# mandt-lab/PSLD

Hardware: NVIDIA B200
Metric: PSLD CIFAR-10 samples/sec (SSCS sampler) (higher is better)
Workload: dtype bf16x3

## Files before the change

### psld_b200/csrc/capi.cu

```cuda

#include <stdarg.h>
#include <string.h>

#include "common.cuh"

namespace psld {

static thread_local char g_err[512] = "";

void set_error(const char* fmt, ...) {
  va_list ap;
  va_start(ap, fmt);
  vsnprintf(g_err, sizeof(g_err), fmt, ap);
  va_end(ap);
}

static int op_launch_count(const psld_op& op) {
  switch (op.kind) {
    case PSLD_OP_LAYOUT: return 1;
    case PSLD_OP_TEMB: return 4;
    case PSLD_OP_GN:
      return (op.in[4] && (op.i[PSLD_GN_C2] == 0 || op.in[5])) ? 1 : 2;
    case PSLD_OP_FIR: return 1;
    case PSLD_OP_CONV: return 1;
    case PSLD_OP_ATTN: return 1;
    case PSLD_OP_AXPBY: return 1;
    default: return 0;
  }
}

static int dispatch(const psld_op& op, cudaStream_t s) {
  switch (op.kind) {
    case PSLD_OP_LAYOUT: return run_layout(op, s);
    case PSLD_OP_TEMB: return run_temb(op, s);
    case PSLD_OP_GN: return run_gn(op, s);
    case PSLD_OP_FIR: return run_fir(op, s);
    case PSLD_OP_CONV:
      if (op.engine == PSLD_ENGINE_TC_GN) return run_conv_gn_tc(op, s);
      return op.engine == PSLD_ENGINE_TC ? run_conv_tc(op, s) : run_conv_simt(op, s);
    case PSLD_OP_ATTN:
      return op.engine == PSLD_ENGINE_TC ? run_attn_tc(op, s) : run_attn_simt(op, s);
    case PSLD_OP_AXPBY: return run_axpby(op, s);
    case PSLD_OP_ZERO: {
      const size_t bytes = (size_t)op.i[0] | ((size_t)op.i[1] << 31);
      if (bytes == 0) return PSLD_OK;
      PSLD_CHECK_ARG(op.out[0] != nullptr, "zero: null pointer");
      PSLD_CHECK_CUDA(cudaMemsetAsync(op.out[0], 0, bytes, s));
      return PSLD_OK;
    }
    default:
      set_error("unknown op kind %d", op.kind);
      return PSLD_EINVAL;
  }
}

}

using namespace psld;

extern "C" int psld_version(void) { return PSLD_B200_VERSION; }

extern "C" const char* psld_last_error(void) { return g_err; }

extern "C" int psld_device_info(int* sm_count, int* cc_major, int* cc_minor) {
  int dev = 0;
  PSLD_CHECK_CUDA(cudaGetDevice(&dev));
  cudaDeviceProp prop;
  PSLD_CHECK_CUDA(cudaGetDeviceProperties(&prop, dev));
  if (sm_count) *sm_count = prop.multiProcessorCount;
  if (cc_major) *cc_major = prop.major;
  if (cc_minor) *cc_minor = prop.minor;
  return PSLD_OK;
}

extern "C" int psld_axpby(float* out, float a, const float* x, float b, const float* y, int64_t n,
                          psld_stream_t stream) {
  return launch_axpby(out, a, x, b, y, n, (cudaStream_t)stream);
}

extern "C" int psld_op_prepare(psld_op* op) {
  PSLD_CHECK_ARG(op != nullptr, "psld_op_prepare: null op");
  if (op->kind == PSLD_OP_CONV && op->engine == PSLD_ENGINE_TC) return prepare_conv_tc(*op);
  if (op->kind == PSLD_OP_CONV && op->engine == PSLD_ENGINE_TC_GN) return prepare_conv_gn_tc(*op);
  if (op->kind == PSLD_OP_ATTN && op->engine == PSLD_ENGINE_TC) return prepare_attn_tc(*op);
  return PSLD_OK;
}

extern "C" int psld_op_release(psld_op* op) {
  PSLD_CHECK_ARG(op != nullptr, "psld_op_release: null op");
  if (op->kind == PSLD_OP_CONV && op->engine == PSLD_ENGINE_TC) return release_conv_tc(*op);
  if (op->kind == PSLD_OP_CONV && op->engine == PSLD_ENGINE_TC_GN) return release_conv_gn_tc(*op);
  if (op->kind == PSLD_OP_ATTN && op->engine == PSLD_ENGINE_TC) return release_attn_tc(*op);
  return PSLD_OK;
}

extern "C" int psld_op_run(const psld_op* op, psld_stream_t stream) {
  PSLD_CHECK_ARG(op != nullptr, "psld_op_run: null op");
  return dispatch(*op, (cudaStream_t)stream);
}

extern "C" int psld_program_run(const psld_op* ops, int n_ops, psld_stream_t stream) {
  PSLD_CHECK_ARG(ops != nullptr && n_ops >= 0, "psld_program_run: bad program");
  for (int i = 0; i < n_ops; ++i) {
    const int rc = dispatch(ops[i], (cudaStream_t)stream);
    if (rc != PSLD_OK) {
      char inner[400];
      strncpy(inner, g_err, sizeof(inner) - 1);
      inner[sizeof(inner) - 1] = 0;
      set_error("op %d (kind %d): %s", i, ops[i].kind, inner);
      return rc;
    }
  }
  return PSLD_OK;
}

extern "C" int psld_program_launches(const psld_op* ops, int n_ops) {
  if (!ops || n_ops < 0) return 0;
  int n = 0;
  for (int i = 0; i < n_ops; ++i) n += op_launch_count(ops[i]);
  return n;
}

static int run_net(const psld_op* ops, int n_ops, int temb_op, const float* time_ptr,
                   cudaStream_t s, int* step_counter = nullptr) {
  for (int i = 0; i < n_ops; ++i) {
    int rc;
    if (i == temb_op || ops[i].kind == PSLD_OP_TEMB) {
      psld_op t = ops[i];
      t.in[0] = time_ptr;
      t.out[2] = step_counter;
      rc = dispatch(t, s);
    } else {
      rc = dispatch(ops[i], s);
    }
    if (rc != PSLD_OK) return rc;
  }
  return PSLD_OK;
}

extern "C" int psld_sampler_run(const psld_op* ops, int n_ops, const psld_sampler_desc* d,
                                psld_stream_t stream) {
  PSLD_CHECK_ARG(ops && d && n_ops > 0, "psld_sampler_run: null argument");
  PSLD_CHECK_ARG(d->state && d->net_in && d->eps && d->time_table, "psld_sampler_run: null buffer");
  PSLD_CHECK_ARG(d->n_steps >= 0 && d->B > 0 && d->chw > 0 && d->chw % 4 == 0,
                 "psld_sampler_run: bad sizes");
  PSLD_CHECK_ARG(d->temb_op >= 0 && d->temb_op < n_ops && ops[d->temb_op].kind == PSLD_OP_TEMB,
                 "psld_sampler_run: temb_op does not index a TEMB op");
  PSLD_CHECK_ARG(d->sampler == 0 ? d->sscs != nullptr : d->em != nullptr,
                 "psld_sampler_run: missing coefficient table");
  PSLD_CHECK_ARG(!d->denoise || d->den, "psld_sampler_run: denoise needs coefficients");
  PSLD_CHECK_ARG(!(d->record && d->fuse_halves), "psld_sampler_run: record requires fuse_halves=0");
  cudaStream_t s = (cudaStream_t)stream;
  const int64_t per_draw = d->B * 2 * d->chw;
  const size_t state_bytes = (size_t)per_draw * dtype_size(d->state_dtype);
  auto z = [&](int64_t k) -> const float* { return d->noise ? d->noise + k * per_draw : nullptr; };
  const int n = d->n_steps;
  int rc = PSLD_OK;

  const bool graph = d->step_counter != nullptr && d->noise == nullptr && d->record == nullptr &&
                     n > 1 && (d->sampler == 0 ? d->sscs_dev != nullptr : d->em_dev != nullptr);
  if (graph) {
    PSLD_CHECK_ARG(s != nullptr, "psld_sampler_run: graph replay needs a non-default stream");
    const int fuse = d->sampler == 0 ? d->fuse_halves : 0;
    if (d->sampler == 0 && fuse && n > 0) {
      rc = psld_sscs_update(d->state, d->state, d->state_dtype, d->net_in, nullptr, nullptr, nullptr,
                            nullptr, &d->sscs[0], PSLD_STAGE_HALF_A, d->seed, 0, d->B, d->chw, s);
      if (rc) return rc;
    }
    const int n_graph = (d->sampler == 0 && fuse == 1) ? n - 1 : n;
    cudaGraph_t g = nullptr;
    cudaGraphExec_t ge = nullptr;
    PSLD_CHECK_CUDA(cudaStreamBeginCapture(s, cudaStreamCaptureModeThreadLocal));
    rc = PSLD_OK;
    if (d->sampler == 0) {
      if (!fuse)
        rc = launch_sscs_table(d->state, d->state_dtype, d->net_in, nullptr, d->sscs_dev,
                               d->step_counter, PSLD_STAGE_HALF_A, d->seed, d->B, d->chw, s);
      if (!rc) rc = run_net(ops, n_ops, d->temb_op, d->time_table, s, d->step_counter);
      int stages = PSLD_STAGE_SCORE | PSLD_STAGE_HALF_B;
      if (fuse == 1) stages |= PSLD_STAGE_HALF_C;
// ... 77 lines not shown
```

### psld_b200/csrc/common.cuh

```cuda
#pragma once

#include <cuda_bf16.h>
#include <cuda_runtime.h>
#include <stdint.h>
#include <stdio.h>

#include "../../include/psld_b200.h"

namespace psld {

void set_error(const char* fmt, ...);

#define PSLD_CHECK_ARG(cond, ...)            \
  do {                                       \
    if (!(cond)) {                           \
      ::psld::set_error(__VA_ARGS__);        \
      return PSLD_EINVAL;                    \
    }                                        \
  } while (0)

#define PSLD_CHECK_CUDA(expr)                                                          \
  do {                                                                                 \
    cudaError_t _e = (expr);                                                           \
    if (_e != cudaSuccess) {                                                           \
// ... 97 lines not shown
    split_bf2(v.x, v.y, h.x, l.x);
    split_bf2(v.z, v.w, h.y, l.y);
    *reinterpret_cast<uint2*>(p) = h;
    *reinterpret_cast<uint2*>(p + lo) = l;
  }
};

template <typename T>
__device__ __forceinline__ float ld_elt(const T* p, int lo);
template <>
__device__ __forceinline__ float ld_elt<float>(const float* p, int) { return *p; }
template <>
__device__ __forceinline__ float ld_elt<__nv_bfloat16>(const __nv_bfloat16* p, int) {
  return __bfloat162float(*p);
}
template <>
__device__ __forceinline__ float ld_elt<bf16s>(const bf16s* p, int lo) {
  return __bfloat162float(p[0].v) + __bfloat162float(p[lo].v);
}
template <typename T>
__device__ __forceinline__ void st_elt(T* p, float v, int lo);
template <>
__device__ __forceinline__ void st_elt<float>(float* p, float v, int) { *p = v; }
template <>
__device__ __forceinline__ void st_elt<__nv_bfloat16>(__nv_bfloat16* p, float v, int) {
  *p = __float2bfloat16_rn(v);
}
template <>
__device__ __forceinline__ void st_elt<bf16s>(bf16s* p, float v, int lo) {
  const __nv_bfloat16 h = __float2bfloat16_rn(v);
  p[0].v = h;
  p[lo].v = __float2bfloat16_rn(v - __bfloat162float(h));
}

template <typename T>
__device__ __forceinline__ float to_f32(T v);
template <>
__device__ __forceinline__ float to_f32<float>(float v) { return v; }
template <>
__device__ __forceinline__ float to_f32<__nv_bfloat16>(__nv_bfloat16 v) {
  return __bfloat162float(v);
}
template <typename T>
__device__ __forceinline__ T from_f32(float v);
template <>
__device__ __forceinline__ float from_f32<float>(float v) { return v; }
template <>
__device__ __forceinline__ __nv_bfloat16 from_f32<__nv_bfloat16>(float v) {
  return __float2bfloat16_rn(v);
}

__device__ __forceinline__ float silu_f(float x) { return x / (1.0f + expf(-x)); }

static inline size_t dtype_size(int dt) { return dt == PSLD_BF16 ? 2 : (dt == PSLD_F64 ? 8 : 4); }

int run_layout(const psld_op& op, cudaStream_t s);
int run_axpby(const psld_op& op, cudaStream_t s);
int launch_axpby(float* out, float a, const float* x, float b, const float* y, int64_t n,
                 cudaStream_t s);
int run_temb(const psld_op& op, cudaStream_t s);
int run_gn(const psld_op& op, cudaStream_t s);
int run_fir(const psld_op& op, cudaStream_t s);
int run_conv_simt(const psld_op& op, cudaStream_t s);
int run_attn_simt(const psld_op& op, cudaStream_t s);
int prepare_conv_tc(psld_op& op);
int release_conv_tc(psld_op& op);
int run_conv_tc(const psld_op& op, cudaStream_t s);
int prepare_conv_gn_tc(psld_op& op);
int release_conv_gn_tc(psld_op& op);
int run_conv_gn_tc(const psld_op& op, cudaStream_t s);
int prepare_attn_tc(psld_op& op);
int release_attn_tc(psld_op& op);
int run_attn_tc(const psld_op& op, cudaStream_t s);

int launch_step_inc(int* step_ptr, cudaStream_t s);
int launch_sscs_table(void* u, int state_dtype, float* net_in, const float* eps,
                      const psld_sscs_coeffs* table, const int* step_ptr, int stages, uint64_t seed,
                      int64_t B, int64_t chw, cudaStream_t s);
int launch_em_table(void* u, int state_dtype, float* net_in, const float* eps,
                    const psld_score_step* table, const int* step_ptr, uint64_t seed, int64_t B,
                    int64_t chw, cudaStream_t s);

}
```

### psld_b200/csrc/conv_gn_tc.cu

```cuda

#include <cuda.h>

#include <new>

#include "common.cuh"
#include "tc_common.cuh"
#include "conv_tc_common.cuh"

namespace psld {

constexpr int GN_TRANSFORM_WARPS = 8;
constexpr int GN_THREADS = (12 + GN_TRANSFORM_WARPS) * 32;
constexpr int GN_B_STAGES = 4;
constexpr int GN_B_BYTES = 128 * 128;
constexpr int GN_MAX_ROWS = 192;
constexpr int GN_VAR_BYTES = GN_MAX_ROWS * 128;
constexpr int GN_ABUF_BYTES = 3 * GN_VAR_BYTES;
constexpr int GN_STAGING_BYTES = 8 * 2048;
constexpr int GN_ADDV_BYTES = 8 * 256;
constexpr int GN_SMEM_BYTES = 2 * GN_ABUF_BYTES + GN_B_STAGES * GN_B_BYTES + GN_STAGING_BYTES + 256 + GN_ADDV_BYTES + 768;

struct ConvGnParams {
  ConvTcParams c;
  const float* affine;
  int cin;
  int silu;
  int rows_in;
  int w_shift;
  int n_images;
};

struct ConvGnState {
  CUtensorMap a1, a2, b, b2, e1, e2;
  ConvGnParams p;
  int grid;
  bool x3;
};

__device__ __forceinline__ int gn_tap(int t9) {
  const int kx = t9 < 3 ? 1 : (t9 < 6 ? 0 : 2);
  const int ky = t9 < 3 ? t9 : (t9 < 6 ? t9 - 3 : t9 - 6);
  return ky * 3 + kx;
}

__device__ __forceinline__ float silu_fast(float x) {
  const float h = 0.5f * x;
  float t;
  asm("tanh.approx.f32 %0, %1;" : "=f"(t) : "f"(h));
  return fmaf(h, t, h);
}

__global__ void __launch_bounds__(GN_THREADS, 1)
conv_gn_tc_kernel(const __grid_constant__ CUtensorMap tmA1, const __grid_constant__ CUtensorMap tmA2,
                  const __grid_constant__ CUtensorMap tmB, const __grid_constant__ CUtensorMap tmB2,
                  const __grid_constant__ CUtensorMap tmE1,
                  const __grid_constant__ CUtensorMap tmE2, const ConvGnParams gp) {
  const ConvTcParams& p = gp.c;
  extern __shared__ uint8_t smem_raw[];
  pdl_launch_dependents();
  const uint32_t base = (smem_u32(smem_raw) + 1023u) & ~1023u;
  auto abuf = [&](int b) { return base + (uint32_t)b * GN_ABUF_BYTES; };
  const uint32_t bring = base + 2 * GN_ABUF_BYTES;
  const uint32_t stg_base = bring + GN_B_STAGES * GN_B_BYTES;
  const uint32_t bar_base = stg_base + GN_STAGING_BYTES;
  const uint32_t addv_base = bar_base + 256u;
  if (addv_base + GN_ADDV_BYTES > smem_u32(smem_raw) + GN_SMEM_BYTES) __trap();
  auto raw_full = [&](int b) { return bar_base + 8u * b; };
  auto a_ready = [&](int b) { return bar_base + 8u * (2 + b); };
  auto a_empty = [&](int b) { return bar_base + 8u * (4 + b); };
  auto b_full = [&](int s) { return bar_base + 8u * (6 + s); };
  auto b_empty = [&](int s) { return bar_base + 8u * (6 + GN_B_STAGES + s); };
  auto tfull_bar = [&](int s) { return bar_base + 8u * (6 + 2 * GN_B_STAGES + s); };
  auto tempty_bar = [&](int s) { return bar_base + 8u * (8 + 2 * GN_B_STAGES + s); };
  auto c_empty = [&](int b) { return bar_base + 8u * (10 + 2 * GN_B_STAGES + b); };
  const uint32_t tmem_slot = bar_base + 8u * (12 + 2 * GN_B_STAGES);
  volatile uint32_t* tmem_slot_ptr =
      reinterpret_cast<volatile uint32_t*>(smem_raw + (tmem_slot - smem_u32(smem_raw)));
// ... 227 lines not shown
          }
          if (x == Wm) *sptr(R + off) = make_uint4(0u, 0u, 0u, 0u);
        }
        asm volatile("fence.proxy.async.shared::cta;" ::: "memory");
        asm volatile("bar.sync 1, %0;" ::"n"(GN_TRANSFORM_WARPS * 32) : "memory");
        if (tt == 0) mbar_arrive_remote(leader_ready0 + 8u * (uint32_t)buf);
        if (++buf == 2) { buf = 0; ph ^= 1; }
      }
    }
  } else if (warp >= 4) {
    const int quarter = warp & 3;
    const int half = (warp - 4) >> 2;
    const uint32_t leader_tempty0 = mapa_rank(tempty_bar(0), 0);
    int acc = 0;
    uint32_t acc_phase = 0;
    pdl_wait();
    for (int v = unit0; v < p.num_virtual; v += unit_step) {
        int unit, nsub, bn;
        tc_decode_unit(p, v, unit, nsub, bn);
      const int n_tile = nsub < 0 ? unit % p.n_tiles_n : (unit % p.n_tiles_n) * p.n_split + nsub;
      const int m_tile = 2 * (unit / p.n_tiles_n) + (int)rank;
      tc_epilogue_tile<true, 32, false>(
          p, tmem_base, acc, m_tile, n_tile, bn, quarter, half, lane,
          stg_base + (uint32_t)(warp - 4) * 2048u, addv_base + (uint32_t)(warp - 4) * 256u,
          [&]() {
            mbar_wait(tfull_bar(acc), acc_phase);
            tc_fence_after();
          },
          [&]() {
            tc_fence_before();
            __syncwarp();
            if (lane == 0) mbar_arrive_remote_relaxed(leader_tempty0 + 8u * (uint32_t)acc);
          });
      if (++acc == 2) { acc = 0; acc_phase ^= 1; }
    }
  }

  tc_fence_before();
  cluster_sync_all();
  if (warp == 1) {
    tc_fence_after();
    asm volatile("tcgen05.dealloc.cta_group::2.sync.aligned.b32 %0, %1;"
                 ::"r"(tmem_base), "n"(TC_TMEM_COLS) : "memory");
  }
}

constexpr int GX_THREADS = 384;
constexpr int GX_TRANSFORM_WARPS = 4;
constexpr int GX_B_STAGES = 2;
constexpr int GX_B_STAGE = 2 * GN_B_BYTES;
constexpr int GX_ABUF_BYTES = 6 * GN_VAR_BYTES;
constexpr int GX_STAGING_BYTES = 4 * 4096;
constexpr int GX_ADDV_BYTES = 4 * 256;
constexpr int GX_SMEM_BYTES = GX_ABUF_BYTES + GX_B_STAGES * GX_B_STAGE + GX_STAGING_BYTES + 256 + GX_ADDV_BYTES + 768;

__device__ __forceinline__ float silu_x3(float x) { return __fdividef(x, 1.0f + __expf(-x)); }

__global__ void __launch_bounds__(GX_THREADS, 1)
conv_gn_x3_kernel(const __grid_constant__ CUtensorMap tmA1, const __grid_constant__ CUtensorMap tmA2,
                  const __grid_constant__ CUtensorMap tmB, const __grid_constant__ CUtensorMap tmB2,
                  const __grid_constant__ CUtensorMap tmE1, const __grid_constant__ CUtensorMap tmE2,
                  const ConvGnParams gp) {
  const ConvTcParams& p = gp.c;
  extern __shared__ uint8_t smem_raw[];
  pdl_launch_dependents();
  const uint32_t base = (smem_u32(smem_raw) + 1023u) & ~1023u;
  auto var = [&](int v, int pl) { return base + (uint32_t)(2 * v + pl) * GN_VAR_BYTES; };
  auto ext_slot = [&](int k) { return base + 2u * GN_VAR_BYTES + (uint32_t)k * 32768u; };
  const uint32_t bring = base + GX_ABUF_BYTES;
  const uint32_t stg_base = bring + GX_B_STAGES * GX_B_STAGE;
  const uint32_t bar_base = stg_base + GX_STAGING_BYTES;
  const uint32_t addv_base = bar_base + 256u;
  if (addv_base + GX_ADDV_BYTES > smem_u32(smem_raw) + GX_SMEM_BYTES) __trap();
  const uint32_t raw_full = bar_base, c_ready = bar_base + 8u, lr_ready = bar_base + 16u;
  const uint32_t c_empty = bar_base + 24u, lr_empty = bar_base + 32u;
  auto b_full = [&](int s) { return bar_base + 40u + 8u * s; };
  auto b_empty = [&](int s) { return bar_base + 40u + 8u * (GX_B_STAGES + s); };
  auto tfull_bar = [&](int s) { return bar_base + 40u + 8u * (2 * GX_B_STAGES + s); };
  auto tempty_bar = [&](int s) { return bar_base + 40u + 8u * (2 * GX_B_STAGES + 2 + s); };
  const uint32_t tmem_slot = bar_base + 40u + 8u * (2 * GX_B_STAGES + 4);
  auto ext_full = [&](int k) { return tmem_slot + 8u + 8u * k; };
  auto ext_empty = [&](int k) { return tmem_slot + 32u + 8u * k; };
  const uint32_t ext_done = tmem_slot + 56u;
  volatile uint32_t* tmem_slot_ptr =
      reinterpret_cast<volatile uint32_t*>(smem_raw + (tmem_slot - smem_u32(smem_raw)));

  const int warp = threadIdx.x >> 5, lane = threadIdx.x & 31;
  const uint32_t rank = cluster_ctarank();
  const int unit0 = (int)(blockIdx.x >> 1), unit_step = (int)(gridDim.x >> 1);

  if (warp == 0 && lane == 0) {
    asm volatile("prefetch.tensormap [%0];" ::"l"(&tmA1) : "memory");
    asm volatile("prefetch.tensormap [%0];" ::"l"(&tmA2) : "memory");
    asm volatile("prefetch.tensormap [%0];" ::"l"(&tmB) : "memory");
    mbar_init(raw_full, 1);
    mbar_init(c_ready, 2);
    mbar_init(lr_ready, 2);
    mbar_init(c_empty, 1);
    mbar_init(lr_empty, 1);
    for (int k = 0; k < 3; ++k) {
      mbar_init(ext_full(k), 1);
      mbar_init(ext_empty(k), 1);
    }
    mbar_init(ext_done, 1);
    for (int s = 0; s < GX_B_STAGES; ++s) {
      mbar_init(b_full(s), 1);
      mbar_init(b_empty(s), 1);
    }
    for (int b = 0; b < 2; ++b) {
      mbar_init(tfull_bar(b), 1);
      mbar_init(tempty_bar(b), 8);
    }
    asm volatile("fence.mbarrier_init.release.cluster;" ::: "memory");
  }
  if (warp == 1) {
    asm volatile("tcgen05.alloc.cta_group::2.sync.aligned.shared::cta.b32 [%0], %1;"
                 ::"r"(tmem_slot), "n"(TC_TMEM_COLS) : "memory");
    asm volatile("tcgen05.relinquish_alloc_permit.cta_group::2.sync.aligned;" ::: "memory");
  }
  tc_fence_before();
  cluster_sync_all();
  tc_fence_after();
  const uint32_t tmem_base = *tmem_slot_ptr;

  const uint32_t raw_bytes = (uint32_t)gp.rows_in * 128u;
  const int total_chunks = p.kchunks;
// ... 117 lines not shown
              for (int k = 0; k < TC_BLOCK_K / 16; ++k)
                tc_mma_bf16_pair(d_tmem, a_lo + (uint64_t)(2 * k), b_hi + (uint64_t)(2 * k), idesc, 1u);
              tc_commit_pair(b_empty(stage));
              if (t9 == 8) tc_commit_pair(lr_empty);
            }
            __syncwarp();
            if (++stage == GX_B_STAGES) { stage = 0; bph ^= 1; }
          }
          cph ^= 1;
        }
        for (int e = 0; e < p.ext_kchunks; ++e) {
          mbar_wait(ext_full(eslot), eph);
          mbar_wait(b_full(stage), bph);
          tc_fence_after();
          const uint64_t a_hi = make_sw128_desc(ext_slot(eslot));
          const uint64_t a_lo = make_sw128_desc(ext_slot(eslot) + 16384u);
          const uint64_t b_hi = make_sw128_desc(bring + (uint32_t)stage * GX_B_STAGE);
          const uint64_t b_lo = make_sw128_desc(bring + (uint32_t)stage * GX_B_STAGE + GN_B_BYTES);
          if (elect_one()) {
#pragma unroll
            for (int k = 0; k < TC_BLOCK_K / 16; ++k)
              tc_mma_bf16_pair(d_tmem, a_hi + (uint64_t)(2 * k), b_hi + (uint64_t)(2 * k), idesc, 1u);
#pragma unroll
            for (int k = 0; k < TC_BLOCK_K / 16; ++k)
              tc_mma_bf16_pair(d_tmem, a_hi + (uint64_t)(2 * k), b_lo + (uint64_t)(2 * k), idesc, 1u);
#pragma unroll
            for (int k = 0; k < TC_BLOCK_K / 16; ++k)
              tc_mma_bf16_pair(d_tmem, a_lo + (uint64_t)(2 * k), b_hi + (uint64_t)(2 * k), idesc, 1u);
            tc_commit_pair(b_empty(stage));
            tc_commit_pair(ext_empty(eslot));
            if (e == p.ext_kchunks - 1) tc_commit_pair(ext_done);
          }
          __syncwarp();
          if (++stage == GX_B_STAGES) { stage = 0; bph ^= 1; }
          if (++eslot == 3) { eslot = 0; eph ^= 1; }
        }
        if (elect_one()) tc_commit_pair(tfull_bar(acc));
        __syncwarp();
        if (++acc == 2) { acc = 0; acc_phase ^= 1; }
      }
    }
  } else if (warp >= 8) {
    constexpr int TT = GX_TRANSFORM_WARPS * 32;
    constexpr int RSTEP = TT / 8;
    constexpr int ITEMS = (GN_MAX_ROWS + RSTEP - 1) / RSTEP;
    const int tt = (int)threadIdx.x - 8 * 32;
    const int j = tt & 7;
    const int r0 = tt >> 3;
    const uint32_t leader_c = mapa_rank(c_ready, 0), leader_lr = mapa_rank(lr_ready, 0);
    const int Wm = p.W - 1;
    const uint32_t sm0 = smem_u32(smem_raw);
    auto sptr = [&](uint32_t a) { return reinterpret_cast<uint4*>(smem_raw + (a - sm0)); };
    uint32_t ph = 0, tph = 0;
    pdl_wait();
    for (int v = unit0; v < p.num_virtual; v += unit_step) {
        int unit, nsub, bn;
        tc_decode_unit(p, v, unit, nsub, bn);
      const int m_tile = 2 * (unit / p.n_tiles_n) + (int)rank;
      const int n0 = m_tile / p.tiles_y;
      const int y0 = (m_tile % p.tiles_y) * p.BH - 1;
      const bool img_ok = n0 < gp.n_images;
      for (int cc = 0; cc < total_chunks; ++cc) {
        float sc[8], sh[8];
#pragma unroll
        for (int q = 0; q < 8; ++q) { sc[q] = 0.f; sh[q] = 0.f; }
        if (img_ok) {
          const float4* ap = reinterpret_cast<const float4*>(
              gp.affine + ((int64_t)n0 * gp.cin + cc * TC_BLOCK_K + j * 8) * 2);
#pragma unroll
          for (int q = 0; q < 4; ++q) {
            const float4 v = __ldg(ap + q);
            sc[2 * q] = v.x; sh[2 * q] = v.y; sc[2 * q + 1] = v.z; sh[2 * q + 1] = v.w;
          }
        }
        mbar_wait(raw_full, ph);
        const uint32_t Ch = var(0, 0), Cl = var(0, 1);
#pragma unroll 3
        for (int u = 0; u < ITEMS; ++u) {
          const int r = r0 + RSTEP * u;
          if (r >= gp.rows_in) continue;
          const int gy = y0 + (r >> gp.w_shift);
          const bool valid = img_ok && gy >= 0 && gy < p.H;
          const uint32_t off = (uint32_t)r * 128u + (uint32_t)((j ^ (r & 7)) << 4);
          uint4 th = make_uint4(0u, 0u, 0u, 0u), tl = th;
          if (valid) {
            th = *sptr(Ch + off);
            tl = *sptr(Cl + off);
            uint32_t* wh = reinterpret_cast<uint32_t*>(&th);
            uint32_t* wl = reinterpret_cast<uint32_t*>(&tl);
#pragma unroll
            for (int q = 0; q < 4; ++q) {
              const float2 fh = bf2_to_f2(wh[q]), fl = bf2_to_f2(wl[q]);
              float a = fmaf(fh.x + fl.x, sc[2 * q], sh[2 * q]);
              float b = fmaf(fh.y + fl.y, sc[2 * q + 1], sh[2 * q + 1]);
              if (gp.silu) { a = silu_x3(a); b = silu_x3(b); }
              split_bf2(a, b, wh[q], wl[q]);
            }
          }
          *sptr(Ch + off) = th;
          *sptr(Cl + off) = tl;
        }
        asm volatile("fence.proxy.async.shared::cta;" ::: "memory");
        asm volatile("bar.sync 1, %0;" ::"n"(GX_TRANSFORM_WARPS * 32) : "memory");
        if (tt == 0) mbar_arrive_remote(leader_c);
        mbar_wait(lr_empty, ph ^ 1);
        if (cc == 0 && p.ext_kchunks > 0) { mbar_wait(ext_done, tph ^ 1); tph ^= 1; }
#pragma unroll 3
        for (int u = 0; u < ITEMS; ++u) {
          const int r = r0 + RSTEP * u;
          if (r >= gp.rows_in) continue;
          const int x = r & Wm;
          const uint32_t off = (uint32_t)r * 128u + (uint32_t)((j ^ (r & 7)) << 4);
          const uint4 th = *sptr(Ch + off), tl = *sptr(Cl + off);
          const uint4 z = make_uint4(0u, 0u, 0u, 0u);
          if (x < Wm) {
            const int rn = r + 1;
            const uint32_t o2 = (uint32_t)rn * 128u + (uint32_t)((j ^ (rn & 7)) << 4);
            *sptr(var(1, 0) + o2) = th;
            *sptr(var(1, 1) + o2) = tl;
          }
          if (x == 0) { *sptr(var(1, 0) + off) = z; *sptr(var(1, 1) + off) = z; }
          if (x > 0) {
            const int rp = r - 1;
            const uint32_t o2 = (uint32_t)rp * 128u + (uint32_t)((j ^ (rp & 7)) << 4);
            *sptr(var(2, 0) + o2) = th;
            *sptr(var(2, 1) + o2) = tl;
          }
          if (x == Wm) { *sptr(var(2, 0) + off) = z; *sptr(var(2, 1) + off) = z; }
        }
        asm volatile("fence.proxy.async.shared::cta;" ::: "memory");
        asm volatile("bar.sync 1, %0;" ::"n"(GX_TRANSFORM_WARPS * 32) : "memory");
        if (tt == 0) mbar_arrive_remote(leader_lr);
        ph ^= 1;
      }
    }
  } else if (warp >= 4) {
    const int quarter = warp & 3;
    const uint32_t leader_tempty0 = mapa_rank(tempty_bar(0), 0);
    int acc = 0;
    uint32_t acc_phase = 0;
    pdl_wait();
    for (int v = unit0; v < p.num_virtual; v += unit_step) {
        int unit, nsub, bn;
        tc_decode_unit(p, v, unit, nsub, bn);
      const int n_tile = nsub < 0 ? unit % p.n_tiles_n : (unit % p.n_tiles_n) * p.n_split + nsub;
      const int m_tile = 2 * (unit / p.n_tiles_n) + (int)rank;
      const uint32_t stg = stg_base + (uint32_t)(warp - 4) * 4096u;
      const uint32_t addv = addv_base + (uint32_t)(warp - 4) * 256u;
      tc_epilogue_tile<false, 32, false, true>(
          p, tmem_base, acc, m_tile, n_tile, bn, quarter, 0, lane, stg, addv,
          [&]() {
            mbar_wait(tfull_bar(acc), acc_phase);
            tc_fence_after();
          },
          []() {});
      tc_epilogue_tile<false, 32, false, true>(
          p, tmem_base, acc, m_tile, n_tile, bn, quarter, 1, lane, stg, addv, []() {},
          [&]() {
            tc_fence_before();
            __syncwarp();
            if (lane == 0) mbar_arrive_remote_relaxed(leader_tempty0 + 8u * (uint32_t)acc);
          });
      if (++acc == 2) { acc = 0; acc_phase ^= 1; }
    }
  }

  tc_fence_before();
  cluster_sync_all();
  if (warp == 1) {
    tc_fence_after();
    asm volatile("tcgen05.dealloc.cta_group::2.sync.aligned.b32 %0, %1;"
                 ::"r"(tmem_base), "n"(TC_TMEM_COLS) : "memory");
  }
}

static int encode_raw_map(CUtensorMap* tm, const void* ptr, int N, int H, int W, int C, int rows_y) {
  const cuuint64_t dims[4] = {(cuuint64_t)C, (cuuint64_t)W, (cuuint64_t)H, (cuuint64_t)N};
  const cuuint64_t strides[3] = {(cuuint64_t)C * 2, (cuuint64_t)W * C * 2, (cuuint64_t)H * W * C * 2};
  const cuuint32_t box[4] = {(cuuint32_t)TC_BLOCK_K, (cuuint32_t)W, (cuuint32_t)rows_y, 1};
  const cuuint32_t estr[4] = {1, 1, 1, 1};
  return encode_bf16_map(tm, ptr, 4, dims, strides, box, estr, "raw tile");
}

int prepare_conv_gn_tc(psld_op& op) {
  const int N = op.i[PSLD_CONV_N], H = op.i[PSLD_CONV_H], W = op.i[PSLD_CONV_W];
  const int C1 = op.i[PSLD_CONV_C1], C2 = op.i[PSLD_CONV_C2], Cout = op.i[PSLD_CONV_COUT];
  const int KS = op.i[PSLD_CONV_KS];
// ... 25 lines not shown
  int block_n = 0;
  for (int cand : {256, 128, 64})
    if (Cout % cand == 0) { block_n = cand; break; }
  const int BH = 128 / W;
  const int rows_in = (BH + 2) * W;
  if (rows_in > GN_MAX_ROWS) return unsupported("tile rows");
  const int64_t m_tiles = (int64_t)N * (H / BH);
  if (m_tiles < 2) return unsupported("single tile");
  ConvGnState* st = new (std::nothrow) ConvGnState();
  if (!st) { set_error("conv_gn_tc: out of host memory"); return PSLD_ECUDA; }
  st->x3 = x3;
  int rc = encode_raw_map(&st->a1, op.in[0], N, H, W, cm * C1, BH + 2);
  if (rc == PSLD_OK)
    rc = C2 > 0 ? encode_raw_map(&st->a2, op.in[1], N, H, W, cm * C2, BH + 2)
                : encode_raw_map(&st->a2, op.in[0], N, H, W, cm * C1, BH + 2);
  const int E1 = op.i[PSLD_CONV_EXT_C1], E2 = op.i[PSLD_CONV_EXT_C2];
  const bool ext = op.in[8] != nullptr && E1 > 0;
  if (ext && (E1 % TC_BLOCK_K || E2 % TC_BLOCK_K || (E2 > 0 && !op.in[9]))) {
    delete st;
    return unsupported("shortcut extension needs E %% 64 == 0");
  }
  if (rc == PSLD_OK)
    rc = ext ? encode_raw_map(&st->e1, op.in[8], N, H, W, cm * E1, x3 ? BH : BH + 2)
             : encode_raw_map(&st->e1, op.in[0], N, H, W, cm * C1, BH + 2);
  if (rc == PSLD_OK)
    rc = (ext && E2 > 0) ? encode_raw_map(&st->e2, op.in[9], N, H, W, cm * E2, x3 ? BH : BH + 2)
                         : encode_raw_map(&st->e2, op.in[0], N, H, W, cm * C1, BH + 2);
  const int K = 9 * (C1 + C2) + (ext ? E1 + E2 : 0);
  if (rc == PSLD_OK) rc = encode_w_map(&st->b, op.in[4], cm * Cout, K, block_n / 2);
  if (rc != PSLD_OK) { delete st; return rc; }
  ConvGnParams& g = st->p;
  ConvTcParams& p = g.c;
  tc_conv_params(p, op, head, H, W, BH, 1, block_n);
  p.num_tiles = (int)(((m_tiles + 1) / 2) * p.n_tiles_n);
  g.affine = (const float*)op.in[6];
  g.cin = C1 + C2;
  g.silu = op.i[PSLD_CONV_GN_SILU];
  g.rows_in = rows_in;
  g.w_shift = W == 32 ? 5 : 4;
  g.n_images = N;
  const int pairs = sm_count() / 2;
  st->b2 = st->b;
  const int ns = tc_plan_tail_split(p, pairs, 64, !head);
  if (ns > 1) {
    rc = encode_w_map(&st->b2, op.in[4], cm * Cout, K, block_n / ns / 2);
    if (rc != PSLD_OK) { delete st; return rc; }
  }
  st->grid = 2 * (p.num_virtual < pairs ? p.num_virtual : pairs);
  static bool attr_set = false;
  if (!attr_set) {
    cudaError_t e = cudaFuncSetAttribute(conv_gn_tc_kernel, cudaFuncAttributeMaxDynamicSharedMemorySize,
                                         GN_SMEM_BYTES);
    if (e == cudaSuccess)
      e = cudaFuncSetAttribute(conv_gn_x3_kernel, cudaFuncAttributeMaxDynamicSharedMemorySize, GX_SMEM_BYTES);
    if (e != cudaSuccess) {
      set_error("conv_gn_tc: cudaFuncSetAttribute failed: %s", cudaGetErrorString(e));
      delete st;
      return PSLD_ECUDA;
    }
    attr_set = true;
  }
  op.aux = st;
  return PSLD_OK;
}

int release_conv_gn_tc(psld_op& op) {
  if (op.aux) {
    delete (ConvGnState*)op.aux;
    op.aux = nullptr;
  }
  return PSLD_OK;
}

int run_conv_gn_tc(const psld_op& op, cudaStream_t s) {
  const ConvGnState* st = (const ConvGnState*)op.aux;
  PSLD_CHECK_ARG(st != nullptr, "conv_gn_tc: op not prepared (call psld_op_prepare)");
  if (st->x3)
    PSLD_CHECK_CUDA(launch_pdl(conv_gn_x3_kernel, dim3((unsigned)st->grid), dim3(GX_THREADS), GX_SMEM_BYTES,
                               s, 2, st->a1, st->a2, st->b, st->b2, st->e1, st->e2, st->p));
  else
    PSLD_CHECK_CUDA(launch_pdl(conv_gn_tc_kernel, dim3((unsigned)st->grid), dim3(GN_THREADS), GN_SMEM_BYTES,
                               s, 2, st->a1, st->a2, st->b, st->b2, st->e1, st->e2, st->p));
  PSLD_CHECK_LAUNCH();
  return PSLD_OK;
}

}
```

### psld_b200/csrc/net_simt.cu

```cuda

#include "common.cuh"

namespace psld {

template <typename T>
__global__ void __launch_bounds__(256)
nchw_to_nhwc_kernel(const float* __restrict__ in, T* __restrict__ out, int N, int C, int HW,
                    int CP, int CW) {
  pdl_trigger_early();
  pdl_wait();
  const int64_t total = (int64_t)N * CW * HW;
  for (int64_t i = (int64_t)blockIdx.x * blockDim.x + threadIdx.x; i < total;
       i += (int64_t)gridDim.x * blockDim.x) {
    const int c = (int)(i % CW);
    const int64_t r = i / CW;
    const int p = (int)(r % HW);
    const int n = (int)(r / HW);
    st_elt<T>(out + r * (CP * Elt<T>::kMul) + c, c < C ? in[((int64_t)n * C + c) * HW + p] : 0.f, CP);
  }
}

template <typename T>
__global__ void __launch_bounds__(256)
nhwc_to_nchw_kernel(const T* __restrict__ in, float* __restrict__ out, int N, int C, int HW) {
// ... 266 lines not shown
    double ds[VW], dq[VW];
#pragma unroll
    for (int k = 0; k < VW; ++k) { s[k] = 0.f; q[k] = 0.f; ds[k] = 0.0; dq[k] = 0.0; }
    int cnt = 0;
    int p = p0 + tr;
    for (; p + (GN_UNROLL - 1) * rows_per_iter < p1; p += GN_UNROLL * rows_per_iter) {
      float v[GN_UNROLL][8];
#pragma unroll
      for (int u = 0; u < GN_UNROLL; ++u) {
        const T* ptr = src + ((int64_t)n * HW + p + u * rows_per_iter) * ld;
        if (VW == 8) Vec8<T>::load(ptr, v[u], lo);
        else { const float4 t = Vec4<T>::load(ptr, lo); v[u][0] = t.x; v[u][1] = t.y; v[u][2] = t.z; v[u][3] = t.w; }
      }
#pragma unroll
      for (int u = 0; u < GN_UNROLL; ++u)
#pragma unroll
        for (int k = 0; k < VW; ++k) { s[k] += v[u][k]; q[k] = fmaf(v[u][k], v[u][k], q[k]); }
      cnt += GN_UNROLL;
      if (cnt >= 32) {
#pragma unroll
        for (int k = 0; k < VW; ++k) { ds[k] += s[k]; dq[k] += q[k]; s[k] = 0.f; q[k] = 0.f; }
        cnt = 0;
      }
    }
    for (; p < p1; p += rows_per_iter) {
      float v[8];
      const T* ptr = src + ((int64_t)n * HW + p) * ld;
      if (VW == 8) Vec8<T>::load(ptr, v, lo);
      else { const float4 t = Vec4<T>::load(ptr, lo); v[0] = t.x; v[1] = t.y; v[2] = t.z; v[3] = t.w; }
#pragma unroll
      for (int k = 0; k < VW; ++k) { s[k] += v[k]; q[k] = fmaf(v[k], v[k], q[k]); }
    }
    int gprev = c / cpg;
    double as = 0.0, aq = 0.0;
#pragma unroll
    for (int k = 0; k < VW; ++k) {
      const int g = (c + k) / cpg;
      if (g != gprev) {
        atomicAdd(&sh[2 * gprev], as);
        atomicAdd(&sh[2 * gprev + 1], aq);
        as = 0.0; aq = 0.0; gprev = g;
      }
      as += ds[k] + (double)s[k];
      aq += dq[k] + (double)q[k];
    }
    atomicAdd(&sh[2 * gprev], as);
    atomicAdd(&sh[2 * gprev + 1], aq);
  }
  __syncthreads();
  double* dst = part + ((int64_t)n * nchunk + chunk) * 2 * G;
  for (int i = threadIdx.x; i < 2 * G; i += blockDim.x) dst[i] = sh[i];
}

__device__ __forceinline__ void gn_group_sums(const double* __restrict__ mg1,
                                              const double* __restrict__ mg2, int n, int C1, int C2,
                                              int cpg, int g, double& su, double& sq) {
  const int nmg1 = C1 >> 2, nmg2 = C2 >> 2, per = cpg >> 2;
  su = 0.0;
  sq = 0.0;
  for (int k = 0; k < per; ++k) {
    const int m = g * per + k;
    const double2 v = m < nmg1
        ? *reinterpret_cast<const double2*>(mg1 + ((int64_t)n * nmg1 + m) * 2)
        : *reinterpret_cast<const double2*>(mg2 + ((int64_t)n * nmg2 + (m - nmg1)) * 2);
    su += v.x;
    sq += v.y;
  }
}

template <typename TI, typename TO, int VW, int kFast, bool kMicro>
__global__ void __launch_bounds__(256)
gn_apply_kernel(const TI* __restrict__ x1, const TI* __restrict__ x2,
                const double* __restrict__ part, const double* __restrict__ mg1,
                const double* __restrict__ mg2, const float* __restrict__ gamma,
                const float* __restrict__ beta, TO* __restrict__ y, int HW, int C1, int C2, int G,
                int nchunk, int nchunk_apply, float eps, int silu) {
  pdl_trigger_early();
  pdl_wait();
  extern __shared__ float shf[];
  const int n = blockIdx.y, chunk = blockIdx.x;
  const int C = C1 + C2, vpr = C / VW, cpg = C / G;
  for (int g = threadIdx.x; g < G; g += blockDim.x) {
    double su = 0, sq = 0;
    if (kMicro) {
      gn_group_sums(mg1, mg2, n, C1, C2, cpg, g, su, sq);
    } else {
      for (int k = 0; k < nchunk; ++k) {
        const double* src = part + ((int64_t)n * nchunk + k) * 2 * G;
        su += src[2 * g];
        sq += src[2 * g + 1];
      }
    }
    const double cntd = (double)HW * cpg;
    const double mean = su / cntd;
    double var = sq / cntd - mean * mean;
    if (var < 0) var = 0;
    shf[g] = (float)mean;
    shf[G + g] = (float)(1.0 / sqrt(var + (double)eps));
  }
  __syncthreads();
  const int rows_per_iter = blockDim.x / vpr;
  const int tv = threadIdx.x % vpr, tr = threadIdx.x / vpr;
  if (tr >= rows_per_iter) return;
  const int per = (HW + nchunk_apply - 1) / nchunk_apply;
  const int p0 = chunk * per, p1 = min(HW, p0 + per);
  const int c = tv * VW;
  const bool first = c < C1;
  const TI* src = first ? x1 + c : x2 + (c - C1);
  const int lo = first ? C1 : C2;
  const int ld = lo * Elt<TI>::kMul;
  constexpr int MO = Elt<TO>::kMul;
  float sc[VW], bi[VW];
#pragma unroll
  for (int k = 0; k < VW; ++k) {
    const int g = (c + k) / cpg;
    sc[k] = shf[G + g] * gamma[c + k];
    bi[k] = beta[c + k] - sc[k] * shf[g];
  }
  int p = p0 + tr;
  for (; p + (GN_UNROLL - 1) * rows_per_iter < p1; p += GN_UNROLL * rows_per_iter) {
    float v[GN_UNROLL][8];
#pragma unroll
    for (int u = 0; u < GN_UNROLL; ++u) {
      const TI* ptr = src + ((int64_t)n * HW + p + u * rows_per_iter) * ld;
      if (VW == 8) Vec8<TI>::load(ptr, v[u], lo);
      else { const float4 t = Vec4<TI>::load(ptr, lo); v[u][0] = t.x; v[u][1] = t.y; v[u][2] = t.z; v[u][3] = t.w; }
    }
#pragma unroll
    for (int u = 0; u < GN_UNROLL; ++u) {
#pragma unroll
      for (int k = 0; k < VW; ++k) {
        float o = fmaf(v[u][k], sc[k], bi[k]);
        v[u][k] = silu ? silu_t<kFast>(o) : o;
      }
      TO* dst = y + ((int64_t)n * HW + p + u * rows_per_iter) * (C * MO) + c;
      if (VW == 8) Vec8<TO>::store(dst, v[u], C);
      else Vec4<TO>::store(dst, make_float4(v[u][0], v[u][1], v[u][2], v[u][3]), C);
    }
  }
  for (; p < p1; p += rows_per_iter) {
    float v[8];
    const TI* ptr = src + ((int64_t)n * HW + p) * ld;
    if (VW == 8) Vec8<TI>::load(ptr, v, lo);
    else { const float4 t = Vec4<TI>::load(ptr, lo); v[0] = t.x; v[1] = t.y; v[2] = t.z; v[3] = t.w; }
#pragma unroll
    for (int k = 0; k < VW; ++k) {
      float o = fmaf(v[k], sc[k], bi[k]);
      v[k] = silu ? silu_t<kFast>(o) : o;
    }
    TO* dst = y + ((int64_t)n * HW + p) * (C * MO) + c;
    if (VW == 8) Vec8<TO>::store(dst, v, C);
    else Vec4<TO>::store(dst, make_float4(v[0], v[1], v[2], v[3]), C);
  }
}

__global__ void __launch_bounds__(256)
gn_affine_micro_kernel(const double* __restrict__ mg1, const double* __restrict__ mg2,
                       const float* __restrict__ gamma, const float* __restrict__ beta,
                       float* __restrict__ affine, int HW, int C1, int C2, int G, float eps) {
  pdl_trigger_early();
  pdl_wait();
  const int n = blockIdx.x;
  const int C = C1 + C2, cpg = C / G;
  for (int c = threadIdx.x; c < C; c += blockDim.x) {
    double su, sq;
    gn_group_sums(mg1, mg2, n, C1, C2, cpg, c / cpg, su, sq);
    const double cntd = (double)HW * cpg;
    const double mean = su / cntd;
    double var = sq / cntd - mean * mean;
    if (var < 0) var = 0;
    const float rstd = (float)(1.0 / sqrt(var + (double)eps));
    const float sc = rstd * gamma[c];
    affine[((int64_t)n * C + c) * 2] = sc;
    affine[((int64_t)n * C + c) * 2 + 1] = beta[c] - sc * (float)mean;
  }
}

__global__ void __launch_bounds__(256)
gn_affine_kernel(const double* __restrict__ part, const float* __restrict__ gamma,
                 const float* __restrict__ beta, float* __restrict__ affine, int HW, int C, int G,
                 int nchunk, float eps) {
  pdl_trigger_early();
  pdl_wait();
  extern __shared__ float shf[];
  const int n = blockIdx.x;
  const int cpg = C / G;
  for (int g = threadIdx.x; g < G; g += blockDim.x) {
    double su = 0, sq = 0;
    for (int k = 0; k < nchunk; ++k) {
      const double* src = part + ((int64_t)n * nchunk + k) * 2 * G;
      su += src[2 * g];
      sq += src[2 * g + 1];
    }
    const double cntd = (double)HW * cpg;
    const double mean = su / cntd;
    double var = sq / cntd - mean * mean;
    if (var < 0) var = 0;
    shf[g] = (float)mean;
    shf[G + g] = (float)(1.0 / sqrt(var + (double)eps));
  }
  __syncthreads();
  for (int c = threadIdx.x; c < C; c += blockDim.x) {
    const int g = c / cpg;
    const float sc = shf[G + g] * gamma[c];
    affine[((int64_t)n * C + c) * 2] = sc;
    affine[((int64_t)n * C + c) * 2 + 1] = beta[c] - sc * shf[g];
  }
}

int run_gn(const psld_op& op, cudaStream_t s) {
  const int N = op.i[PSLD_GN_N], HW = op.i[PSLD_GN_HW], C1 = op.i[PSLD_GN_C1];
  const int C2 = op.i[PSLD_GN_C2], G = op.i[PSLD_GN_G], silu = op.i[PSLD_GN_SILU];
  const int idt = op.i[PSLD_GN_IN_DTYPE], odt = op.i[PSLD_GN_OUT_DTYPE];
  const int nchunk = op.i[PSLD_GN_NCHUNK];
  const int C = C1 + C2;
  PSLD_CHECK_ARG(N > 0 && HW > 0 && C1 > 0 && C2 >= 0 && G > 0 && nchunk > 0, "gn: bad sizes");
  PSLD_CHECK_ARG(C % G == 0 && C1 % 4 == 0 && C2 % 4 == 0 && C / 4 <= 256,
                 "gn: need C %% G == 0, C1,C2 %% 4 == 0, C <= 1024 (C1=%d C2=%d G=%d)", C1, C2, G);
  PSLD_CHECK_ARG(op.in[0] && (C2 == 0 || op.in[1]) && op.in[2] && op.in[3] && op.out[0] &&
                 op.out[1], "gn: null pointer");
  PSLD_CHECK_ARG(idt == odt, "gn: input and output dtypes must match (%d vs %d)", idt, odt);
  const bool v8 = (C1 % 8 == 0) && (C2 % 8 == 0);
  double* part = (double*)op.out[1];
  const size_t sh1 = 2 * G * sizeof(double), sh2 = 2 * G * sizeof(float);
  const bool fused = op.in[4] && (C2 == 0 || op.in[5]);
  int nchunk_eff = nchunk;
  if (fused) {
// ... 350 lines not shown
```

Baseline: 5.607.

## Fold GroupNorm affine computation into the split-bf16 conv+GN tensor-core kernel

Adds a host-side planner that detects a GN affine-only op whose table feeds only the next conv_gn_tc op, then launches a templated conv kernel that computes per-group mean/rstd from micro-group sums. Each tile's moments go into a double-buffered shared slot, and the next tile's moments are prefetched during the last K chunk. This removes one kernel launch and the affine table round trip per fold, in exchange for extra per-tile moment math in the transform warps and a per-call planning pass with a hash map on the host.

New measurement: 5.516, median of 6. 1.6% lower.

```diff
diff --git a/psld_b200/csrc/capi.cu b/psld_b200/csrc/capi.cu
--- a/psld_b200/csrc/capi.cu
+++ b/psld_b200/csrc/capi.cu
@@ -1,6 +1,9 @@
 
 #include <stdarg.h>
 #include <string.h>
+
+#include <unordered_map>
+#include <vector>
 
 #include "common.cuh"
 
@@ -54,6 +57,31 @@
   }
 }
 
+static void plan_gn_folds(const psld_op* ops, int n_ops, std::vector<char>& fold) {
+  fold.assign((size_t)n_ops, 0);
+  auto writes_table = [&](int j, const void* t) {
+    return j >= 0 && ops[j].kind == PSLD_OP_GN && ops[j].i[PSLD_GN_AFFINE_ONLY] && ops[j].out[0] == t;
+  };
+  std::unordered_map<const void*, bool> private_table;
+  for (int j = 0; j < n_ops; ++j) {
+    const psld_op& o = ops[j];
+    for (int k = 0; k < PSLD_OP_NP; ++k) {
+      if (o.in[k]) {
+        const bool ok = k == 6 && o.kind == PSLD_OP_CONV && o.engine == PSLD_ENGINE_TC_GN &&
+                        writes_table(j - 1, o.in[k]);
+        auto it = private_table.emplace(o.in[k], true).first;
+        it->second = it->second && ok;
+      }
+      if (o.out[k]) {
+        auto it = private_table.emplace(o.out[k], true).first;
+        it->second = it->second && k == 0 && writes_table(j, o.out[k]);
+      }
+    }
+  }
+  for (int i = 0; i + 1 < n_ops; ++i)
+    if (conv_gn_tc_can_fold(ops[i], ops[i + 1]) && private_table[ops[i].out[0]]) fold[(size_t)i] = 1;
+}
+
 }
 
 using namespace psld;
@@ -101,8 +129,11 @@
 
 extern "C" int psld_program_run(const psld_op* ops, int n_ops, psld_stream_t stream) {
   PSLD_CHECK_ARG(ops != nullptr && n_ops >= 0, "psld_program_run: bad program");
+  std::vector<char> fold;
+  plan_gn_folds(ops, n_ops, fold);
   for (int i = 0; i < n_ops; ++i) {
-    const int rc = dispatch(ops[i], (cudaStream_t)stream);
+    const int rc = fold[i] ? run_conv_gn_tc_folded(ops[i + 1], ops[i], (cudaStream_t)stream)
+                           : dispatch(ops[i], (cudaStream_t)stream);
     if (rc != PSLD_OK) {
       char inner[400];
       strncpy(inner, g_err, sizeof(inner) - 1);
@@ -110,22 +141,30 @@
       set_error("op %d (kind %d): %s", i, ops[i].kind, inner);
       return rc;
     }
+    i += fold[i];
   }
   return PSLD_OK;
 }
 
 extern "C" int psld_program_launches(const psld_op* ops, int n_ops) {
   if (!ops || n_ops < 0) return 0;
+  std::vector<char> fold;
+  plan_gn_folds(ops, n_ops, fold);
   int n = 0;
-  for (int i = 0; i < n_ops; ++i) n += op_launch_count(ops[i]);
+  for (int i = 0; i < n_ops; ++i) n += fold[i] ? 0 : op_launch_count(ops[i]);
   return n;
 }
 
 static int run_net(const psld_op* ops, int n_ops, int temb_op, const float* time_ptr,
                    cudaStream_t s, int* step_counter = nullptr) {
+  std::vector<char> fold;
+  plan_gn_folds(ops, n_ops, fold);
   for (int i = 0; i < n_ops; ++i) {
     int rc;
-    if (i == temb_op || ops[i].kind == PSLD_OP_TEMB) {
+    if (fold[i]) {
+      rc = run_conv_gn_tc_folded(ops[i + 1], ops[i], s);
+      ++i;
+    } else if (i == temb_op || ops[i].kind == PSLD_OP_TEMB) {
       psld_op t = ops[i];
       t.in[0] = time_ptr;
       t.out[2] = step_counter;
diff --git a/psld_b200/csrc/common.cuh b/psld_b200/csrc/common.cuh
--- a/psld_b200/csrc/common.cuh
+++ b/psld_b200/csrc/common.cuh
@@ -173,6 +173,42 @@
 
 __device__ __forceinline__ float silu_f(float x) { return x / (1.0f + expf(-x)); }
 
+__device__ __forceinline__ void gn_group_sums(const double* __restrict__ mg1,
+                                              const double* __restrict__ mg2, int n, int C1, int C2,
+                                              int cpg, int g, double& su, double& sq) {
+  const int nmg1 = C1 >> 2, nmg2 = C2 >> 2, per = cpg >> 2;
+  su = 0.0;
+  sq = 0.0;
+#pragma unroll 4
+  for (int k = 0; k < per; ++k) {
+    const int m = g * per + k;
+    const double2 v = m < nmg1
+        ? *reinterpret_cast<const double2*>(mg1 + ((int64_t)n * nmg1 + m) * 2)
+        : *reinterpret_cast<const double2*>(mg2 + ((int64_t)n * nmg2 + (m - nmg1)) * 2);
+    su += v.x;
+    sq += v.y;
+  }
+}
+
+__device__ __forceinline__ void gn_group_moments(const double* __restrict__ mg1,
+                                                 const double* __restrict__ mg2, int n, int C1, int C2,
+                                                 int cpg, int g, int HW, float eps, float& rstd,
+                                                 float& mean_f) {
+  double su, sq;
+  gn_group_sums(mg1, mg2, n, C1, C2, cpg, g, su, sq);
+  const double cntd = (double)HW * cpg;
+  const double mean = su / cntd;
+  double var = sq / cntd - mean * mean;
+  if (var < 0) var = 0;
+  rstd = (float)(1.0 / sqrt(var + (double)eps));
+  mean_f = (float)mean;
+}
+
+__device__ __forceinline__ float2 gn_channel_affine(float rstd, float mean_f, float gamma, float beta) {
+  const float sc = rstd * gamma;
+  return make_float2(sc, beta - sc * mean_f);
+}
+
 static inline size_t dtype_size(int dt) { return dt == PSLD_BF16 ? 2 : (dt == PSLD_F64 ? 8 : 4); }
 
 int run_layout(const psld_op& op, cudaStream_t s);
@@ -190,6 +226,8 @@
 int prepare_conv_gn_tc(psld_op& op);
 int release_conv_gn_tc(psld_op& op);
 int run_conv_gn_tc(const psld_op& op, cudaStream_t s);
+bool conv_gn_tc_can_fold(const psld_op& gn, const psld_op& conv);
+int run_conv_gn_tc_folded(const psld_op& conv, const psld_op& gn, cudaStream_t s);
 int prepare_attn_tc(psld_op& op);
 int release_attn_tc(psld_op& op);
 int run_attn_tc(const psld_op& op, cudaStream_t s);
diff --git a/psld_b200/csrc/conv_gn_tc.cu b/psld_b200/csrc/conv_gn_tc.cu
--- a/psld_b200/csrc/conv_gn_tc.cu
+++ b/psld_b200/csrc/conv_gn_tc.cu
@@ -23,6 +23,12 @@
 struct ConvGnParams {
   ConvTcParams c;
   const float* affine;
+  const double* mg1;
+  const double* mg2;
+  const float* gamma;
+  const float* beta;
+  int gn_c1, gn_c2, cpg, groups, hw;
+  float eps;
   int cin;
   int silu;
   int rows_in;
@@ -356,10 +362,40 @@
 constexpr int GX_ABUF_BYTES = 6 * GN_VAR_BYTES;
 constexpr int GX_STAGING_BYTES = 4 * 4096;
 constexpr int GX_ADDV_BYTES = 4 * 256;
-constexpr int GX_SMEM_BYTES = GX_ABUF_BYTES + GX_B_STAGES * GX_B_STAGE + GX_STAGING_BYTES + 256 + GX_ADDV_BYTES + 768;
+constexpr int GX_MOM_BYTES = 2 * 32 * 8;
+constexpr int GX_SMEM_BYTES = GX_ABUF_BYTES + GX_B_STAGES * GX_B_STAGE + GX_STAGING_BYTES + 256 + GX_ADDV_BYTES +
+                              GX_MOM_BYTES + 768;
+
+__device__ __forceinline__ void gn_write_moments(const ConvGnParams& gp, int n, int lane, float2* slot) {
+  if (lane < gp.groups) {
+    float rstd, mean;
+    gn_group_moments(gp.mg1, gp.mg2, n, gp.gn_c1, gp.gn_c2, gp.cpg, lane, gp.hw, gp.eps, rstd, mean);
+    slot[lane] = make_float2(rstd, mean);
+  }
+}
+
+__device__ __forceinline__ void gn_fold_affine(const ConvGnParams& gp, const float2* slot, int c0,
+                                               float (&sc)[8], float (&sh)[8]) {
+  const int g0 = c0 / gp.cpg;
+  const int split = (g0 + 1) * gp.cpg - c0;
+  const float2 a0 = slot[g0], a1 = slot[min(g0 + 1, gp.groups - 1)];
+  const float4* gq = reinterpret_cast<const float4*>(gp.gamma + c0);
+  const float4* bq = reinterpret_cast<const float4*>(gp.beta + c0);
+  const float4 ga = __ldg(gq), gb = __ldg(gq + 1), ba = __ldg(bq), bb = __ldg(bq + 1);
+  const float gam[8] = {ga.x, ga.y, ga.z, ga.w, gb.x, gb.y, gb.z, gb.w};
+  const float bet[8] = {ba.x, ba.y, ba.z, ba.w, bb.x, bb.y, bb.z, bb.w};
+#pragma unroll
+  for (int q = 0; q < 8; ++q) {
+    const float2 m = q >= split ? a1 : a0;
+    const float2 a = gn_channel_affine(m.x, m.y, gam[q], bet[q]);
+    sc[q] = a.x;
+    sh[q] = a.y;
+  }
+}
 
 __device__ __forceinline__ float silu_x3(float x) { return __fdividef(x, 1.0f + __expf(-x)); }
 
+template <bool kFold>
 __global__ void __launch_bounds__(GX_THREADS, 1)
 conv_gn_x3_kernel(const __grid_constant__ CUtensorMap tmA1, const __grid_constant__ CUtensorMap tmA2,
                   const __grid_constant__ CUtensorMap tmB, const __grid_constant__ CUtensorMap tmB2,
@@ -375,7 +411,8 @@
   const uint32_t stg_base = bring + GX_B_STAGES * GX_B_STAGE;
   const uint32_t bar_base = stg_base + GX_STAGING_BYTES;
   const uint32_t addv_base = bar_base + 256u;
-  if (addv_base + GX_ADDV_BYTES > smem_u32(smem_raw) + GX_SMEM_BYTES) __trap();
+  const uint32_t mom_base = addv_base + GX_ADDV_BYTES;
+  if (mom_base + (kFold ? GX_MOM_BYTES : 0) > smem_u32(smem_raw) + GX_SMEM_BYTES) __trap();
   const uint32_t raw_full = bar_base, c_ready = bar_base + 8u, lr_ready = bar_base + 16u;
   const uint32_t c_empty = bar_base + 24u, lr_empty = bar_base + 32u;
   auto b_full = [&](int s) { return bar_base + 40u + 8u * s; };
@@ -599,6 +636,8 @@
     const uint32_t sm0 = smem_u32(smem_raw);
     auto sptr = [&](uint32_t a) { return reinterpret_cast<uint4*>(smem_raw + (a - sm0)); };
     uint32_t ph = 0, tph = 0;
+    float2* mom = reinterpret_cast<float2*>(smem_raw + (mom_base - sm0));
+    int tile_k = 0;
     pdl_wait();
     for (int v = unit0; v < p.num_virtual; v += unit_step) {
         int unit, nsub, bn;
@@ -607,11 +646,17 @@
       const int n0 = m_tile / p.tiles_y;
       const int y0 = (m_tile % p.tiles_y) * p.BH - 1;
       const bool img_ok = n0 < gp.n_images;
+      if (kFold && v == unit0) {
+        if (tt < 32 && img_ok) gn_write_moments(gp, n0, tt, mom);
+        asm volatile("bar.sync 1, %0;" ::"n"(GX_TRANSFORM_WARPS * 32) : "memory");
+      }
       for (int cc = 0; cc < total_chunks; ++cc) {
         float sc[8], sh[8];
 #pragma unroll
         for (int q = 0; q < 8; ++q) { sc[q] = 0.f; sh[q] = 0.f; }
-        if (img_ok) {
+        if (kFold && img_ok) {
+          gn_fold_affine(gp, mom + 32 * (tile_k & 1), cc * TC_BLOCK_K + j * 8, sc, sh);
+        } else if (img_ok) {
           const float4* ap = reinterpret_cast<const float4*>(
               gp.affine + ((int64_t)n0 * gp.cin + cc * TC_BLOCK_K + j * 8) * 2);
 #pragma unroll
@@ -650,6 +695,12 @@
         asm volatile("fence.proxy.async.shared::cta;" ::: "memory");
         asm volatile("bar.sync 1, %0;" ::"n"(GX_TRANSFORM_WARPS * 32) : "memory");
         if (tt == 0) mbar_arrive_remote(leader_c);
+        if (kFold && cc == total_chunks - 1 && tt < 32 && v + unit_step < p.num_virtual) {
+          int un, nsn, bnn;
+          tc_decode_unit(p, v + unit_step, un, nsn, bnn);
+          const int nn = (2 * (un / p.n_tiles_n) + (int)rank) / p.tiles_y;
+          if (nn < gp.n_images) gn_write_moments(gp, nn, tt, mom + 32 * ((tile_k + 1) & 1));
+        }
         mbar_wait(lr_empty, ph ^ 1);
         if (cc == 0 && p.ext_kchunks > 0) { mbar_wait(ext_done, tph ^ 1); tph ^= 1; }
 #pragma unroll 3
@@ -680,6 +731,7 @@
         if (tt == 0) mbar_arrive_remote(leader_lr);
         ph ^= 1;
       }
+      ++tile_k;
     }
   } else if (warp >= 4) {
     const int quarter = warp & 3;
@@ -811,7 +863,9 @@
     cudaError_t e = cudaFuncSetAttribute(conv_gn_tc_kernel, cudaFuncAttributeMaxDynamicSharedMemorySize,
                                          GN_SMEM_BYTES);
     if (e == cudaSuccess)
-      e = cudaFuncSetAttribute(conv_gn_x3_kernel, cudaFuncAttributeMaxDynamicSharedMemorySize, GX_SMEM_BYTES);
+      e = cudaFuncSetAttribute(conv_gn_x3_kernel<false>, cudaFuncAttributeMaxDynamicSharedMemorySize, GX_SMEM_BYTES);
+    if (e == cudaSuccess)
+      e = cudaFuncSetAttribute(conv_gn_x3_kernel<true>, cudaFuncAttributeMaxDynamicSharedMemorySize, GX_SMEM_BYTES);
     if (e != cudaSuccess) {
       set_error("conv_gn_tc: cudaFuncSetAttribute failed: %s", cudaGetErrorString(e));
       delete st;
@@ -831,17 +885,58 @@
   return PSLD_OK;
 }
 
+static int launch_conv_gn(const ConvGnState* st, const ConvGnParams& gp, bool fold, cudaStream_t s) {
+  if (fold)
+    PSLD_CHECK_CUDA(launch_pdl(conv_gn_x3_kernel<true>, dim3((unsigned)st->grid), dim3(GX_THREADS), GX_SMEM_BYTES,
+                               s, 2, st->a1, st->a2, st->b, st->b2, st->e1, st->e2, gp));
+  else if (st->x3)
+    PSLD_CHECK_CUDA(launch_pdl(conv_gn_x3_kernel<false>, dim3((unsigned)st->grid), dim3(GX_THREADS), GX_SMEM_BYTES,
+                               s, 2, st->a1, st->a2, st->b, st->b2, st->e1, st->e2, gp));
+  else
+    PSLD_CHECK_CUDA(launch_pdl(conv_gn_tc_kernel, dim3((unsigned)st->grid), dim3(GN_THREADS), GN_SMEM_BYTES,
+                               s, 2, st->a1, st->a2, st->b, st->b2, st->e1, st->e2, gp));
+  PSLD_CHECK_LAUNCH();
+  return PSLD_OK;
+}
+
 int run_conv_gn_tc(const psld_op& op, cudaStream_t s) {
   const ConvGnState* st = (const ConvGnState*)op.aux;
   PSLD_CHECK_ARG(st != nullptr, "conv_gn_tc: op not prepared (call psld_op_prepare)");
-  if (st->x3)
-    PSLD_CHECK_CUDA(launch_pdl(conv_gn_x3_kernel, dim3((unsigned)st->grid), dim3(GX_THREADS), GX_SMEM_BYTES,
-                               s, 2, st->a1, st->a2, st->b, st->b2, st->e1, st->e2, st->p));
-  else
-    PSLD_CHECK_CUDA(launch_pdl(conv_gn_tc_kernel, dim3((unsigned)st->grid), dim3(GN_THREADS), GN_SMEM_BYTES,
-                               s, 2, st->a1, st->a2, st->b, st->b2, st->e1, st->e2, st->p));
-  PSLD_CHECK_LAUNCH();
-  return PSLD_OK;
-}
-
-}
+  return launch_conv_gn(st, st->p, false, s);
+}
+
+bool conv_gn_tc_can_fold(const psld_op& gn, const psld_op& conv) {
+  if (gn.kind != PSLD_OP_GN || !gn.i[PSLD_GN_AFFINE_ONLY] || conv.kind != PSLD_OP_CONV ||
+      conv.engine != PSLD_ENGINE_TC_GN || conv.i[PSLD_CONV_IN_DTYPE] != PSLD_BF16S || !conv.aux ||
+      !gn.out[0] || conv.in[6] != gn.out[0])
+    return false;
+  const int C1 = gn.i[PSLD_GN_C1], C2 = gn.i[PSLD_GN_C2], G = gn.i[PSLD_GN_G];
+  const int C = C1 + C2;
+  if (!gn.in[4] || (C2 > 0 && !gn.in[5]) || !gn.in[2] || !gn.in[3]) return false;
+  if (C1 <= 0 || C2 < 0 || C1 % 4 || C2 % 4 || G <= 0 || G > 32 || C % G || (C / G) % 4) return false;
+  if (((uintptr_t)gn.in[2] | (uintptr_t)gn.in[3]) % 16) return false;
+  return gn.i[PSLD_GN_N] == conv.i[PSLD_CONV_N] &&
+         C == conv.i[PSLD_CONV_C1] + conv.i[PSLD_CONV_C2] &&
+         gn.i[PSLD_GN_HW] == conv.i[PSLD_CONV_H] * conv.i[PSLD_CONV_W];
+}
+
+int run_conv_gn_tc_folded(const psld_op& conv, const psld_op& gn, cudaStream_t s) {
+  const ConvGnState* st = (const ConvGnState*)conv.aux;
+  PSLD_CHECK_ARG(st != nullptr, "conv_gn_tc: op not prepared (call psld_op_prepare)");
+  ConvGnParams gp = st->p;
+  gp.affine = nullptr;
+  gp.mg1 = (const double*)gn.in[4];
+  gp.mg2 = (const double*)gn.in[5];
+  gp.gamma = (const float*)gn.in[2];
+  gp.beta = (const float*)gn.in[3];
+  gp.gn_c1 = gn.i[PSLD_GN_C1];
+  gp.gn_c2 = gn.i[PSLD_GN_C2];
+  gp.groups = gn.i[PSLD_GN_G];
+  gp.cpg = (gp.gn_c1 + gp.gn_c2) / gp.groups;
+  gp.hw = gn.i[PSLD_GN_HW];
+  gp.eps = gn.f[0];
+  PSLD_CHECK_ARG(st->x3, "conv_gn_tc: GroupNorm fold needs split-bf16 operands");
+  return launch_conv_gn(st, gp, true, s);
+}
+
+}
diff --git a/psld_b200/csrc/net_simt.cu b/psld_b200/csrc/net_simt.cu
--- a/psld_b200/csrc/net_simt.cu
+++ b/psld_b200/csrc/net_simt.cu
@@ -342,22 +342,6 @@
   for (int i = threadIdx.x; i < 2 * G; i += blockDim.x) dst[i] = sh[i];
 }
 
-__device__ __forceinline__ void gn_group_sums(const double* __restrict__ mg1,
-                                              const double* __restrict__ mg2, int n, int C1, int C2,
-                                              int cpg, int g, double& su, double& sq) {
-  const int nmg1 = C1 >> 2, nmg2 = C2 >> 2, per = cpg >> 2;
-  su = 0.0;
-  sq = 0.0;
-  for (int k = 0; k < per; ++k) {
-    const int m = g * per + k;
-    const double2 v = m < nmg1
-        ? *reinterpret_cast<const double2*>(mg1 + ((int64_t)n * nmg1 + m) * 2)
-        : *reinterpret_cast<const double2*>(mg2 + ((int64_t)n * nmg2 + (m - nmg1)) * 2);
-    su += v.x;
-    sq += v.y;
-  }
-}
-
 template <typename TI, typename TO, int VW, int kFast, bool kMicro>
 __global__ void __launch_bounds__(256)
 gn_apply_kernel(const TI* __restrict__ x1, const TI* __restrict__ x2,
@@ -453,16 +437,11 @@
   const int n = blockIdx.x;
   const int C = C1 + C2, cpg = C / G;
   for (int c = threadIdx.x; c < C; c += blockDim.x) {
-    double su, sq;
-    gn_group_sums(mg1, mg2, n, C1, C2, cpg, c / cpg, su, sq);
-    const double cntd = (double)HW * cpg;
-    const double mean = su / cntd;
-    double var = sq / cntd - mean * mean;
-    if (var < 0) var = 0;
-    const float rstd = (float)(1.0 / sqrt(var + (double)eps));
-    const float sc = rstd * gamma[c];
-    affine[((int64_t)n * C + c) * 2] = sc;
-    affine[((int64_t)n * C + c) * 2 + 1] = beta[c] - sc * (float)mean;
+    float rstd, mean;
+    gn_group_moments(mg1, mg2, n, C1, C2, cpg, c / cpg, HW, eps, rstd, mean);
+    const float2 a = gn_channel_affine(rstd, mean, gamma[c], beta[c]);
+    affine[((int64_t)n * C + c) * 2] = a.x;
+    affine[((int64_t)n * C + c) * 2 + 1] = a.y;
   }
 }
 
```
